# TINY-KE/DSP-SLAM-RGBD

Hardware: AMD Instinct MI355X
Metric: object-reconstructions/sec (2048 pts, 10 GN iters) (higher is better)
Workload: dtype fp16-mfma: 3xFP16 split (hi/lo fp16, fp32 accumulate) for every value that reaches an output + one-product fp16 classification of ray samples

## Files before the change

### dsp-slam-rgbd_amd/csrc/dsr_api.hip

```cpp
#include <hip/hip_runtime.h>
#include <rccl/rccl.h>
#include <dlfcn.h>

#include <algorithm>
#include <chrono>
#include <climits>
#include <cmath>
#include <cstdio>
#include <cstring>
#include <functional>
#include <map>
#include <mutex>
#include <string>
#include <thread>
#include <vector>

#include "../../include/dsr.h"
#include "dsr_kernels.hpp"
#include "dsr_mc.hpp"
#include "dsr_mesh.hpp"

#ifndef DSR_DEFAULT_FWD_VARIANT
#define DSR_DEFAULT_FWD_VARIANT 12
#endif
// ... 1443 lines not shown
  if (timing) DSR_CHECK(ctx, hipEventRecord(b->ev[0], ctx->stream));
  hipLaunchKernelGGL(k_init_state, dim3(n), dim3(64), 0, ctx->stream, n, b->t_in, b->is_oc, b->z_in, b->st,
                     b->zbuf, b->iters);
  DSR_CHECK(ctx, hipMemsetAsync(b->diag, 0, sizeof(int) * STD_INTS, ctx->stream));
  if (b->n_tied) DSR_CHECK(ctx, hipMemsetAsync(b->fail_view, 0xff, sizeof(int) * b->n_tied, ctx->stream));
  if (b->tie_multi)
    for (const auto& gr : b->groups)
      hipLaunchKernelGGL(k_views_pose, dim3(gr.nt), dim3(64), 0, ctx->stream, (const int2*)b->tie + gr.t0,
                         b->st + gr.o0, (const float*)b->cview + (size_t)gr.o0 * 16);
  b->spare_run = false;
  return batch_enqueue_iters(b, timing, 0, b->iters);
}

static int batch_redo(dsr_batch* b) {
  dsr_ctx* ctx = b->ctx;
  if (b->loop_iters <= b->iters || b->spare_run) return 0;
  std::vector<ObjState> hs(b->n_obj);
  DSR_CHECK(ctx, hipMemcpy(hs.data(), b->st, sizeof(ObjState) * hs.size(), hipMemcpyDeviceToHost));
  bool any = false;
  for (const ObjState& o : hs) any = any || (o.status == ST_RUNNING && o.lite_redo);
  if (!any) return 0;
  b->spare_run = true;
  const int rc = batch_enqueue_iters(b, b->timed, b->iters, b->loop_iters);
  if (rc) return rc;
  DSR_CHECK(ctx, hipEventRecord(b->done_ev, ctx->stream));
  return 1;
}
static int batch_finish(dsr_batch* b) {
  dsr_ctx* ctx = b->ctx;
  std::lock_guard<std::recursive_mutex> run(ctx->run_mu);
  DSR_CHECK(ctx, hipStreamSynchronize(ctx->stream));
  const int rc = batch_redo(b);
  if (rc < 0) return rc;
  if (rc == 1) DSR_CHECK(ctx, hipStreamSynchronize(ctx->stream));
  return 0;
}

static int batch_enqueue_iters(dsr_batch* b, bool timing, int it0, int it1) {
  dsr_ctx* ctx = b->ctx;
  hipStream_t s0 = ctx->stream;
  const int n = b->n_obj;
  const DevDecoder& D = b->dec->D;
  const GNParams P = b->P;
  const int grid = ctx->n_cu;
  const int cb = (n + 63) / 64;
  const int fv = fwd_variant();
  const FwdKernel fwdk = fwd_kernel_for(D, fv);
  const JacKernel jack = jac_kernel_for(D);
  const LiteKernel litek = lite_kernel();
  {
    const int fl = fv & 15;
    const bool known = fl == 1 || fl == 2 || fl == 3 || fl == 6 || fl == 7 || fl == 8 || fl == 12;
    const int jv = jac_variant();
    b->ran_fwd = is_variant(D) ? 12 : (known ? fv : (fv & ~15));
    b->ran_jac = is_variant(D) ? 12 : ((jv == 8 || jv == 12) ? jv : 0);
    b->ran_lite = b->lite ? lite_variant_dispatched() : 0;
    b->ran_ring = is_variant(D) ? 2 : split_ring();
  }
  const int np = (int)b->passes.size() - 1;
  const size_t epi = ev_per_iter(b);
  const int G = (int)b->groups.size();
  DSR_CHECK(ctx, hipEventRecord(b->fork_ev, s0));
  for (int g = 1; g < G; ++g) DSR_CHECK(ctx, hipStreamWaitEvent(ctx->gstream[g], b->fork_ev, 0));
  for (int it = it0; it < it1; ++it) {
    for (int g = 0; g < G; ++g) {
      const dsr_batch::Group& gr = b->groups[g];
      hipStream_t s = ctx->gstream[g];
      const int ng = gr.n, o0 = gr.o0;
      const ObjDesc* desc = b->desc + o0;
      ObjState* st = b->st + o0;
      float* zbuf = b->zbuf + (size_t)o0 * CODE;
      float* b0 = b->bias0f + (size_t)o0 * HID;
      float* b4 = b->bias4f + (size_t)o0 * HID;
      hipEvent_t* ev = b->ev.data() + 2 + ((size_t)it * G + g) * epi;
      hipLaunchKernelGGL(k_iter_begin, dim3(ng), dim3(512), 0, s, ng, desc, st, zbuf, D, P, b0, b4, b->dobs);
      ErtArgs ert = b->lite_cfg;
      ert.dead = b->dead;
      ert.M = b->M;
      ert.nth = -P.cut_off;
      ert.st = b->lite ? st : nullptr;
      ert.refine = b->refine;
      ert.diag = b->diag;
      const bool chunked = b->prescan && gr.n_rch > 0;
      if (!chunked)
        DSR_CHECK(ctx, hipMemsetD32Async(reinterpret_cast<hipDeviceptr_t>(b->dense + gr.c0), 0x7fc00000,
                                         (size_t)(gr.c1 - gr.c0), s));
      for (int pz = 0; pz < np; ++pz) {
        const int ra = b->passes[pz], rb = b->passes[pz + 1];
        if (chunked) {
          if (pz == 0)
            hipLaunchKernelGGL(k_sample_scan, dim3(gr.n_rch), dim3(RENDER_RAYS), 0, s, gr.rchunks, desc, st, b->rays,
                               b->M, rb, b->dead, b->rinfo, b->rwin, gr.scnt, b->dense);
          else
            hipLaunchKernelGGL(k_sample_count, dim3(gr.n_rch), dim3(RENDER_RAYS), 0, s, gr.rchunks, desc, st, b->rays,
                               b->M, ra, rb, b->dead, b->rinfo, b->rwin, gr.scnt);
          hipLaunchKernelGGL(k_sample_emit, dim3(gr.n_rch + 1), dim3(RENDER_RAYS), 0, s, gr.rchunks, desc, st,
                             b->rays, b->M, ra, rb, b->cand, b->rwin, gr.scnt,
                             ChunkTiles{gr.och, gr.tiles_f, gr.nt_f, ng, b->lite ? LTILE : TILE, 0});
        } else {
          hipLaunchKernelGGL(k_sample_pass, dim3(ng), dim3(SAMPLE_THREADS), 0, s, ng, desc, st, b->rays, b->M,
                             ra, rb, b->cand, b->dead, b->rinfo);
          hipLaunchKernelGGL(k_tiles_fwd, dim3(1), dim3(1024), 0, s, ng, desc, st, gr.tiles_f, gr.nt_f,
                             b->lite ? LTILE : TILE, 0);
        }
        if (fv & 1) DSR_CHECK(ctx, hipMemsetAsync(gr.sync, 0, 8 * 32 * sizeof(unsigned), s));
        if (timing) DSR_CHECK(ctx, hipEventRecord(ev[2 * pz], s));
        if (b->lite)
          hipLaunchKernelGGL(litek, dim3(grid), dim3(512), 0, s, D, gr.tiles_f, gr.nt_f, desc,
                             b->cand, b0, b4, b->dense, ert);
        else
          hipLaunchKernelGGL(fwdk, dim3(grid), dim3(512), 0, s, D, gr.tiles_f, gr.nt_f, desc, b->cand,
                             b0, b4, b->dense, gr.sync, ert, MaskArgs{nullptr, nullptr, nullptr, nullptr});
        if (timing) DSR_CHECK(ctx, hipEventRecord(ev[2 * pz + 1], s));
      }
      const bool rays = gr.n_rch > 0;
      if (b->lite) {
        if (rays) {
          hipLaunchKernelGGL(k_refine_scan, dim3(gr.n_rch), dim3(REFINE_SCAN_THREADS), 0, s, gr.rchunks, desc, st, b->M,
                             b->refine, refine_all() ? nullptr : b->dense, -P.cut_off, b->rbits, b->abits, gr.ccnt,
                             b->ma.slotmap);
          const int wp = (b->ma.pts && fv == 12) ? 1 : 0;
          hipLaunchKernelGGL(k_refine_emit, dim3(gr.n_rch + (chunked ? 1 : 0)), dim3(RENDER_RAYS), 0, s, gr.rchunks,
                             desc, st, b->rays, b->M, b->cand, b->ma.slotmap, b->rbits, b->abits, gr.ccnt,
                             chunked ? ChunkTiles{gr.och, gr.tiles_f, gr.nt_f, ng, TILE, wp} : ChunkTiles{});
        }
        if (!chunked)
          hipLaunchKernelGGL(k_tiles_fwd, dim3(1), dim3(1024), 0, s, ng, desc, st, gr.tiles_f, gr.nt_f, TILE,
                             (b->ma.pts && fv == 12) ? 1 : 0);
        if (timing) DSR_CHECK(ctx, hipEventRecord(ev[2 * np], s));
        const ErtArgs ex{nullptr, b->M, -P.cut_off, st, nullptr};
        if (b->ma.msk && fv == 12)
          hipLaunchKernelGGL(fwd16_kernel<512>(), dim3(grid), dim3(512), 0, s, D, gr.tiles_f, gr.nt_f, desc,
                             b->cand, b0, b4, b->dense, gr.sync, ex, b->ma);
        else
          hipLaunchKernelGGL(fwdk, dim3(grid), dim3(512), 0, s, D, gr.tiles_f, gr.nt_f, desc, b->cand,
                             b0, b4, b->dense, gr.sync, ex, MaskArgs{nullptr, nullptr, nullptr, nullptr});
        if (timing) DSR_CHECK(ctx, hipEventRecord(ev[2 * np + 1], s));
      }
      const bool keep = b->lite && b->ma.msk && fv == 12;
      const int je = 2 * (np + (b->lite ? 1 : 0));
      if (rays) {
        hipLaunchKernelGGL(k_render_rays, dim3(gr.n_rch), dim3(RENDER_RAYS), render_lds_bytes(b->M), s,
                           gr.rchunks, desc, st, b->rays, b->dobs, P, b->dense, b->kst, b->rst,
                           keep ? b->sst : nullptr, (const int*)b->ma.slotmap, gr.ccnt);
        hipLaunchKernelGGL(k_render_gather, dim3(gr.n_rch + (chunked ? 1 : 0)), dim3(256), 0, s, gr.rchunks, desc,
                           st, gr.ccnt, b->M, b->kst, b->rst, b->sst, b->kpts, b->kres, keep ? b->kslot : nullptr,
                           chunked ? ChunkTiles{gr.och, gr.tiles_j, gr.nt_j, ng, TILE, 0} : ChunkTiles{});
      }
      if (!chunked)
        hipLaunchKernelGGL(k_tiles_jac, dim3(1), dim3(1024), 0, s, ng, desc, st, gr.tiles_j, gr.nt_j);
      if (timing) DSR_CHECK(ctx, hipEventRecord(ev[je], s));
      hipLaunchKernelGGL(jack, dim3(grid), dim3(512), 0, s, D, gr.tiles_j, gr.nt_j, desc, st,
                         b->pts, b->kpts, b->kres, b0, b4, P, b->slots,
                         (const float4*)nullptr, (float*)nullptr, (float*)nullptr,
                         keep ? b->ma : MaskArgs{nullptr, nullptr, nullptr, nullptr},
                         D.ln_mask ? ctx->lnws[g] : (float*)nullptr);
      if (timing) DSR_CHECK(ctx, hipEventRecord(ev[je + 1], s));
      float* sred = b->sred + (size_t)o0 * SRED_STRIDE;
      hipLaunchKernelGGL(k_reduce_slots, dim3(ng * SLOT_BLOCKS), dim3(256), 0, s, desc, st, b->slots, sred, it,
                         b->counts + (size_t)o0 * COUNT_STRIDE, n);
      if (b->n_tied) {
        hipLaunchKernelGGL(k_solve_views, dim3(gr.nt), dim3(SOLVE_THREADS), 0, s, (const int2*)b->tie + gr.t0, desc,
                           st, zbuf, P, sred, b->tr_H ? b->tr_H + (size_t)o0 * TRACE_H_STRIDE : nullptr,
                           b->tr_v ? b->tr_v + (size_t)o0 * TRACE_V_STRIDE : nullptr,
                           b->tr_i ? b->tr_i + (size_t)o0 * TRACE_I_STRIDE : nullptr, n, b->fail_view + gr.t0);
        if (b->tie_multi)
          hipLaunchKernelGGL(k_views_pose, dim3(gr.nt), dim3(64), 0, s, (const int2*)b->tie + gr.t0, st,
                             (const float*)b->cview + (size_t)o0 * 16);
        continue;
      }
      hipLaunchKernelGGL(k_solve, dim3(ng), dim3(SOLVE_THREADS), 0, s, ng, desc, st, zbuf, P, sred,
                         b->tr_H ? b->tr_H + (size_t)o0 * TRACE_H_STRIDE : nullptr,
                         b->tr_v ? b->tr_v + (size_t)o0 * TRACE_V_STRIDE : nullptr,
                         b->tr_i ? b->tr_i + (size_t)o0 * TRACE_I_STRIDE : nullptr, n);
    }
  }
  for (int g = 1; g < G; ++g) {
    DSR_CHECK(ctx, hipEventRecord(b->join_ev[g], ctx->gstream[g]));
    DSR_CHECK(ctx, hipStreamWaitEvent(s0, b->join_ev[g], 0));
  }
  hipLaunchKernelGGL(k_finalize, dim3(cb), dim3(64), 0, s0, n, b->st, b->zbuf, b->out);
  DSR_CHECK(ctx, hipGetLastError());
  if (timing) DSR_CHECK(ctx, hipEventRecord(b->ev[1], s0));
  return 0;
// ... 1345 lines not shown
```

### dsp-slam-rgbd_amd/csrc/dsr_kernels.hpp

```cpp
#pragma once
#include "dsr_dev.hpp"
#include "dsr_mlp.hpp"
#include "dsr_mlp16.hpp"
#include "dsr_mlp_lite.hpp"
#include "../../include/dsr.h"

extern "C" __device__ __attribute__((const)) unsigned long long __ockl_wfred_max_u64(unsigned long long);

namespace dsr {

template <int N>
__device__ __forceinline__ void lu_small(float (&a)[N][N], int (&piv)[N]) {
#pragma unroll
  for (int k = 0; k < N; ++k) {
    int p = k;
    float best = fabsf(a[k][k]);
#pragma unroll
    for (int r = k + 1; r < N; ++r)
      if (fabsf(a[r][k]) > best) { best = fabsf(a[r][k]); p = r; }
    piv[k] = p;
#pragma unroll
    for (int r = k + 1; r < N; ++r) {
      const bool sw = (p == r);
#pragma unroll
// ... 537 lines not shown
        cnt = walk_count(make_float3(rp[0], rp[1], rp[2]), L, M, ra, rb, true, nin);
      }
    }
    rwin[d.ray_off + ray] = cnt | ((j0 + 1) << 8);
#ifdef DSR_EXP_PROV
    prov_alive(S.iters_done, ra, d.ray_off + ray, alive ? cnt + 1 : -1);
    prov_emit(S.iters_done, ra, d.ray_off + ray, cnt > 0 ? (j0 >= 0 ? j0 + ra : -2) : -1);
#endif
  }
  chunk_sums(cnt, 0, sc + 2 * blockIdx.x);
}

__global__ __launch_bounds__(RENDER_RAYS) DSR_NO_PK_F32 void k_sample_emit(const RenderChunk* __restrict__ chunks,
                                                             const ObjDesc* __restrict__ desc, ObjState* st,
                                                             const float* __restrict__ rays_all, int M, int ra,
                                                             int rb, float4* __restrict__ cand,
                                                             const int* __restrict__ rwin,
                                                             const int* __restrict__ sc, ChunkTiles T) {
  if (T.och && (int)blockIdx.x == (int)gridDim.x - 1) {
    chunk_tiles_fwd(T, desc, st, sc, 2, ra == 0 ? sc + 1 : nullptr);
    return;
  }
  const RenderChunk ch = chunks[blockIdx.x];
  ObjState& S = st[ch.obj];
  if (S.status != ST_RUNNING) return;
  const ObjDesc d = desc[ch.obj];
  __shared__ int wsum[RENDER_RAYS / 64];
  __shared__ SampleLds L;
  const int tid = threadIdx.x, lane = tid & 63, wv = tid >> 6;
  stage_samples(L, S, M, tid);
  const bool last = (int)blockIdx.x == ch.first + ch.n - 1;
  const int base = block_chunk_sum(sc, 2, ch.first, blockIdx.x);
  const int nin = (last && ra == 0) ? block_chunk_sum(sc + 1, 2, ch.first, blockIdx.x + 1) : 0;
  const int ray = ch.ray0 + tid;
  int cnt = 0, j0 = -1;
  float3 rv = make_float3(0.f, 0.f, 0.f);
  if (ray < d.n_rays) {
    const int w = rwin[d.ray_off + ray];
    cnt = w & 255;
    j0 = (w >> 8) - 1;
    if (cnt > 0) {
      const float* rp = rays_all + (size_t)(d.ray_off + ray) * 3;
      rv = make_float3(rp[0], rp[1], rp[2]);
    }
  }
  const int inc = wave_incl_scan(cnt, lane);
  if (lane == 63) wsum[wv] = inc;
  __syncthreads();
  int off = d.cand_off + base + inc - cnt;
  for (int k = 0; k < wv; ++k) off += wsum[k];
  if (cnt > 0 && j0 >= 0) {
    for (int k = ra; k < ra + cnt; ++k) {
      const float3 x = ray_sample(rv, L, j0 + k);
      cand[off++] = make_float4(x.x, x.y, x.z, __int_as_float(ray * M + j0 + k));
    }
  } else if (cnt > 0) {
    int rank = 0;
    for (int j = 0; j < M && rank < rb; ++j) {
      const float3 x = ray_sample(rv, L, j);
      const float nrm = sqrtf((x.x * x.x + x.y * x.y) + x.z * x.z);
      if (!(nrm < 1.0f)) continue;
      if (rank >= ra) cand[off++] = make_float4(x.x, x.y, x.z, __int_as_float(ray * M + j));
      ++rank;
    }
  }
  if (tid == 0 && last) {
    int t = base;
    for (int k = 0; k < RENDER_RAYS / 64; ++k) t += wsum[k];
    S.n_emit = t;
    S.n_eval += t;
    if (ra == 0) {
      S.n_valid = nin;
      if (nin < 10) {
        S.status = ST_FAIL;
        S.fail_reason = DSR_FAIL_RENDER_FEW;
      }
    }
  }
}

__global__ __launch_bounds__(SAMPLE_THREADS) DSR_NO_PK_F32 void k_sample_pass(int n_obj, const ObjDesc* __restrict__ desc,
                                                                ObjState* st, const float* __restrict__ rays_all,
                                                                int M, int ra, int rb, float4* __restrict__ cand,
                                                                int* __restrict__ dead, int* __restrict__ rinfo) {
  const int o = blockIdx.x;
  ObjState& S = st[o];
  if (S.status != ST_RUNNING) return;
  const ObjDesc d = desc[o];
  const float* rays = rays_all + (size_t)d.ray_off * 3;
  const bool first = ra == 0;
  __shared__ int wsum[SAMPLE_THREADS / 64];
  __shared__ int wnin[SAMPLE_THREADS / 64];
  __shared__ int base_s, nin_s;
  __shared__ SampleLds L;
  const int tid = threadIdx.x, lane = tid & 63, wv = tid >> 6;
  if (tid == 0) { base_s = 0; nin_s = 0; }
  stage_samples(L, S, M, tid);
  __syncthreads();
  for (int r0 = 0; r0 < d.n_rays; r0 += SAMPLE_THREADS) {
    const int ray = r0 + tid;
    int cnt = 0, nin = 0;
    int j0 = -1;
    float3 rv = make_float3(0.f, 0.f, 0.f);
    if (ray < d.n_rays) {
      rv = make_float3(rays[ray * 3 + 0], rays[ray * 3 + 1], rays[ray * 3 + 2]);
      if (first) dead_put(dead + d.ray_off + ray, 0);
      const bool alive = first || dead_get(dead + d.ray_off + ray) == 0;
      if (alive && !first) {
        const int info = rinfo[d.ray_off + ray];
        if (info >= 0) {
          j0 = info & 255;
          nin = info >> 8;
          cnt = max(0, min(rb, nin) - ra);
        }
      }
      if (alive && j0 < 0) {
        if (first) {
          int rank = 0, jf = -1, jl = -1;
          for (int j = 0; j < M; ++j) {
            const float3 x = ray_sample(rv, L, j);
            const float nrm = sqrtf((x.x * x.x + x.y * x.y) + x.z * x.z);
            if (!(nrm < 1.0f)) continue;
            if (jf < 0) jf = j;
            jl = j;
            if (rank < rb) ++cnt;
            ++rank;
          }
          nin = rank;
          rinfo[d.ray_off + ray] = rank == 0 ? 0 : (jl - jf + 1 == rank ? (jf | (rank << 8)) : -1);
        } else {
          cnt = walk_count(rv, L, M, ra, rb, true, nin);
        }
      }
    }
    const int inc = wave_incl_scan(cnt, lane);
    int nin_w = nin;
#pragma unroll
    for (int k = 32; k > 0; k >>= 1) nin_w += __shfl_xor(nin_w, k);
    if (lane == 63) wsum[wv] = inc;
    if (lane == 0) wnin[wv] = nin_w;
    __syncthreads();
    int off = base_s + inc - cnt;
    for (int k = 0; k < wv; ++k) off += wsum[k];
    if (cnt > 0 && j0 >= 0) {
      for (int k = ra; k < ra + cnt; ++k) {
        const float3 x = ray_sample(rv, L, j0 + k);
        cand[d.cand_off + off++] = make_float4(x.x, x.y, x.z, __int_as_float(ray * M + j0 + k));
      }
    } else if (cnt > 0) {
      int rank = 0;
      for (int j = 0; j < M && rank < rb; ++j) {
        const float3 x = ray_sample(rv, L, j);
        const float nrm = sqrtf((x.x * x.x + x.y * x.y) + x.z * x.z);
        if (!(nrm < 1.0f)) continue;
        if (rank >= ra) cand[d.cand_off + off++] = make_float4(x.x, x.y, x.z, __int_as_float(ray * M + j));
        ++rank;
      }
    }
    __syncthreads();
    if (tid == 0) {
      int t = 0, u = 0;
      for (int k = 0; k < SAMPLE_THREADS / 64; ++k) { t += wsum[k]; u += wnin[k]; }
      base_s += t;
      nin_s += u;
    }
    __syncthreads();
  }
  if (tid == 0) {
    S.n_emit = base_s;
    S.n_eval += base_s;
    if (first) {
// ... 657 lines not shown
  const int w = __builtin_amdgcn_readfirstlane(threadIdx.x >> 6);
  float* const lnw = lnws ? lnws + (size_t)blockIdx.x * LN_WS_WG : nullptr;
  const int nt = *n_tiles;
#ifdef DSR_EXP_STAMP
  unsigned long long jstamp[8] = {0, 0, 0, 0, 0, 0, 0, 0};
  unsigned long long jstamp_last = __builtin_amdgcn_s_memtime();
  int jtiles = 0;
#endif
  for (int ti = blockIdx.x; ti < nt; ti += gridDim.x) {
    const Tile tl = tiles[ti];
    const ObjDesc d = desc[tl.obj];
#ifdef DSR_EXP_STAMP
    ++jtiles;
#endif
    float zpre = 0.f;
    {
      const int tid = opaque(threadIdx.x);
      if (tid < TILE) {
        float x = 0.f, y = 0.f, z = 0.f, aux = 0.f, rr = 0.f;
        zpre = bias0f[tl.obj * HID];
        if (tid < tl.count) {
          if (tl.term == 0) {
            const float* p = pts_all + (size_t)(d.pts_off + tl.start + tid) * 3;
            const float3 xo = xform(st[tl.obj].T, p[0], p[1], p[2]);
            x = xo.x; y = xo.y; z = xo.z;
          } else if (tl.term == 1) {
            const float4 v = kpts[d.cand_off + tl.start + tid];
            x = v.x; y = v.y; z = v.z; aux = v.w;
            rr = kres[d.cand_off + tl.start + tid];
          } else {
            const float4 v = raw_pts[tl.start + tid];
            x = v.x; y = v.y; z = v.z;
          }
        }
        *reinterpret_cast<float4*>(sm.xyz + tid * 4) = make_float4(x, y, z, aux);
        sm.r[tid] = rr;
      }
    }
    __syncthreads();
    uint64_t mk[8];
    float v[4][4][4];
    floatx4 acc[4][4];
    int sa;
    Scales2 fs;
    bool fast = false;
    if (MA.kslot != nullptr && tl.term == 1) {
      const int tid = opaque(threadIdx.x);
      int bad = 0;
      if (tid < tl.count) bad = MA.kslot[d.cand_off + tl.start + tid] < 0;
      fast = !__syncthreads_or(bad);
    } else if (MA.pts != nullptr && tl.term == 0) {
      fast = true;
    }
    auto mslot = [&](int p) {
      return tl.term == 1 ? d.cand_off + MA.kslot[d.cand_off + tl.start + p] : MA.surf_base + d.pts_off + tl.start + p;
    };
    if (fast) {
      const int lane = opaque(threadIdx.x & 63), g = lane >> 4, c = lane & 15;
#pragma unroll
      for (int l = 0; l < 8; ++l) mk[l] = 0;
#pragma unroll
      for (int cb = 0; cb < 4; ++cb) {
        const int p = 16 * cb + c;
        if (p < tl.count) {
          const uint4 m4 = *reinterpret_cast<const uint4*>(MA.msk + (size_t)mslot(p) * 256 + (w * 4 + g) * 8);
          const unsigned dw[4] = {m4.x, m4.y, m4.z, m4.w};
#pragma unroll
          for (int l = 0; l < 8; ++l) {
            const unsigned u = (dw[l >> 1] >> (16 * (l & 1))) & 0xFFFFu;
#pragma unroll
            for (int q = 0; q < 4; ++q) mk[l] |= (uint64_t)((u >> (4 * q)) & 0xFu) << (16 * q + 4 * cb);
          }
        }
      }
      const int tid = opaque(threadIdx.x);
      if (tid < TILE) sm.y[tid] = (tid < tl.count) ? MA.yv[mslot(tid)] : 0.f;
      __syncthreads();
      JSTAMP(0)
    } else {
      JSTAMP(0)
      {
        const int lane = opaque(threadIdx.x & 63), g = lane >> 4, c = lane & 15;
        const float* bias0 = bias0f + tl.obj * HID;
        float m = 0.f;
        mk[0] = 0;
#pragma unroll
        for (int q = 0; q < 4; ++q) {
          const int n0 = 64 * w + 16 * q + 4 * g;
          const float4 bb = *reinterpret_cast<const float4*>(bias0 + n0);
          float wx[12];
#pragma unroll
          for (int i = 0; i < 12; ++i) wx[i] = D.W0x[n0 * 3 + i];
#pragma unroll
          for (int cb = 0; cb < 4; ++cb) {
            const float4 p = *reinterpret_cast<const float4*>(sm.xyz + (16 * cb + c) * 4);
#pragma unroll
            for (int r = 0; r < 4; ++r)
              v[q][cb][r] = fetch4(bb, r) + ((wx[3 * r] * p.x + wx[3 * r + 1] * p.y) + wx[3 * r + 2] * p.z);
          }
        }
        if (VAR && (D.ln_mask & 1)) ln_fwd(v, D.ln_g[0], D.ln_b[0], D.ln_dim[0], sm.red, sm.red2, w, lane, lnw);
#pragma unroll
        for (int q = 0; q < 4; ++q)
#pragma unroll
          for (int cb = 0; cb < 4; ++cb)
#pragma unroll
            for (int r = 0; r < 4; ++r) {
              const float h = fmaxf(v[q][cb][r], 0.f);
              if (h > 0.f) mk[0] |= 1ull << ((q * 4 + cb) * 4 + r);
              v[q][cb][r] = h;
              m = fmaxf(m, h);
            }
        if (VAR && D.xyz_all && w == 7) xyz_rows(v, sm.xyz, lane, m, 3);
        JSTAMP(7)
        fs = block_scale2(m, sm.wmax, w, lane);
        JSTAMP(3)
        write_split(v, fs.of(w), sm.Hh, sm.Hl, w, lane);
        JSTAMP(4)
      }
      __syncthreads();
      JSTAMP(5)
#pragma unroll 1
      for (int l = 1; l <= 6; ++l) {
        const int lane = opaque(threadIdx.x & 63), g = lane >> 4;
        gemm16_sel<PRIO, NB, JFWD_LS>(D.Wh_raw[l], w, D.Kf[l] / 32, sm.Hh, sm.Hl, acc, lane, fs.resc());
        JSTAMP(1)
        const float usc = ldexpf(1.f, -(D.sw[l] + fs.b));
        const float* bias = (l == 4) ? bias4f + tl.obj * HID : D.bias[l];
        float m = 0.f;
        uint64_t bits = 0;
        if (VAR && ((D.ln_mask >> l) & 1)) {
#pragma unroll
          for (int q = 0; q < 4; ++q) {
            const float4 bb = *reinterpret_cast<const float4*>(bias + 64 * w + 16 * q + 4 * g);
#pragma unroll
            for (int cb = 0; cb < 4; ++cb)
#pragma unroll
              for (int r = 0; r < 4; ++r) v[q][cb][r] = __builtin_fmaf(accr(acc[q][cb], r), usc * rc_sign(q, cb), fetch4(bb, r));
          }
          ln_fwd(v, D.ln_g[l], D.ln_b[l], D.ln_dim[l], sm.red, sm.red2, w, lane, lnw + (size_t)l * LN_WS_LAYER);
#pragma unroll
          for (int q = 0; q < 4; ++q)
#pragma unroll
            for (int cb = 0; cb < 4; ++cb)
#pragma unroll
              for (int r = 0; r < 4; ++r) {
                const float h = fmaxf(v[q][cb][r], 0.f);
                if (h > 0.f) bits |= 1ull << ((q * 4 + cb) * 4 + r);
                v[q][cb][r] = h;
                m = fmaxf(m, h);
              }
        } else {
#pragma unroll
        for (int q = 0; q < 4; ++q) {
          const float4 bb = *reinterpret_cast<const float4*>(bias + 64 * w + 16 * q + 4 * g);
#pragma unroll
          for (int cb = 0; cb < 4; ++cb) {
#pragma unroll
            for (int r = 0; r < 4; ++r) {
              const float h = fmaxf(__builtin_fmaf(accr(acc[q][cb], r), usc * rc_sign(q, cb), fetch4(bb, r)), 0.f);
              if (h > 0.f) bits |= 1ull << ((q * 4 + cb) * 4 + r);
              v[q][cb][r] = h;
              m = fmaxf(m, h);
            }
          }
        }
        }
        mk[l] = bits;
        {
          const int xr = VAR ? xyz_row(D, l) : (l == 3 ? D.l3 : -1);
          if (xr >= 0 && w == (xr >> 6)) xyz_rows(v, sm.xyz, lane, m, (xr >> 4) & 3);
        }
        JSTAMP(2)
        fs = block_scale2(m, sm.wmax, w, lane);
        JSTAMP(3)
        write_split(v, fs.of(w), sm.Hh, sm.Hl, w, lane);
        JSTAMP(4)
        __syncthreads();
        JSTAMP(5)
      }
      {
        const int lane = opaque(threadIdx.x & 63);
        gemm16_sel<PRIO, NB, JFWD_LS>(D.Wh_raw[7], w, D.Kf[7] / 32, sm.Hh, sm.Hl, acc, lane, fs.resc());
        JSTAMP(1)
        const int un = D.sw[7] + fs.b;
#pragma unroll
        for (int q = 0; q < 4; ++q)
#pragma unroll
          for (int cb = 0; cb < 4; ++cb)
#pragma unroll
            for (int r = 0; r < 4; ++r) acc[q][cb][r] = ldexpf(acc[q][cb][r], -un) * rc_sign(q, cb);
        const bool ln7 = VAR && ((D.ln_mask >> 7) & 1);
        if (ln7) ln_l7(acc, D, sm.red, sm.red2, w, lane, lnw + (size_t)7 * LN_WS_LAYER);
        epi_l7(acc, D, sm.red, w, lane, mk[7], VAR ? sm.xyz : nullptr, !ln7);
      }
      __syncthreads();
      {
        const int tid = opaque(threadIdx.x);
        if (tid < TILE) {
          float s = sm.red[tid];
          for (int k = 1; k < NWAVE; ++k) s += sm.red[k * TILE + tid];
          float y = tanhf(s + D.b8);
          if (VAR && D.use_tanh) y = tanhf(y);
          sm.y[tid] = y;
        }
      }
      __syncthreads();
    }
    float xg[4][3] = {{0.f, 0.f, 0.f}, {0.f, 0.f, 0.f}, {0.f, 0.f, 0.f}, {0.f, 0.f, 0.f}};
    const bool xlane = VAR && D.xyz_all && w == 7 && ((threadIdx.x & 63) >> 4) == 3;
    {
      const int lane = opaque(threadIdx.x & 63), g = lane >> 4, c = lane & 15;
      float m = 0.f;
#pragma unroll
      for (int q = 0; q < 4; ++q) {
        const int n0 = 64 * w + 16 * q + 4 * g;
        const float4 w8 = *reinterpret_cast<const float4*>(D.W8 + n0);
#pragma unroll
        for (int cb = 0; cb < 4; ++cb) {
          const int p = 16 * cb + c;
          const float yy = sm.y[p];
          float dt = 1.f - yy * yy;
          if (VAR && D.use_tanh) {
            const float t = atanhf(yy);
            dt = dt * (1.f - t * t);
          }
#pragma unroll
          for (int r = 0; r < 4; ++r) {
            const float gv = ((mk[7] >> ((q * 4 + cb) * 4 + r)) & 1ull) ? dt * fetch4(w8, r) : 0.f;
            v[q][cb][r] = gv;
            m = fmaxf(m, fabsf(gv));
            if (q == 3 && r >= 1 && xlane) xg[cb][r - 1] = dt * fetch4(w8, r);
          }
        }
      }
      if (VAR && ((D.ln_mask >> 7) & 1))
        m = ln_bwd(v, D.ln_g[7], D.ln_dim[7], sm.red, sm.red2, w, lane, lnw + (size_t)7 * LN_WS_LAYER);
      JSTAMP(7)
      sa = block_scale(m, sm.wmax, w, lane);
      JSTAMP(3)
      write_split(v, sa, sm.Hh, sm.Hl, w, lane);
      JSTAMP(4)
    }
    __syncthreads();
    JSTAMP(5)
#pragma unroll 1
    for (int l = 7; l >= 1; --l) {
      const int lane = opaque(threadIdx.x & 63), g = lane >> 4, c = lane & 15;
      gemm16_sel<PRIO, NB, BWD_LS>(D.Wbh_raw[l], w, D.Kb[l] / 32, sm.Hh, sm.Hl, acc, lane);
      JSTAMP(1)
      const float usc = ldexpf(1.f, -(D.swb[l] + sa));
// ... 755 lines not shown
```

### dsp-slam-rgbd_amd/csrc/dsr_mlp16.hpp

```cpp
#pragma once
#include <utility>
#include "dsr_dev.hpp"
#include "dsr_mlp.hpp"

namespace dsr {

typedef _Float16 half8 __attribute__((ext_vector_type(8)));
typedef _Float16 half4 __attribute__((ext_vector_type(4)));

constexpr int PH = 528;

#if defined(DSR_LITE_EXPERIMENTS) || defined(DSR_EXP_NOSIGN)
constexpr bool SPLIT_ROW_SIGNS = false;
#else
constexpr bool SPLIT_ROW_SIGNS = true;
#endif
__device__ __forceinline__ constexpr float row_sign(int q) { return (SPLIT_ROW_SIGNS && (q & 1)) ? -1.f : 1.f; }
#ifdef DSR_EXP_COLSIGN
__device__ __forceinline__ constexpr float col_sign(int cb) { return (SPLIT_ROW_SIGNS && (cb & 1)) ? -1.f : 1.f; }
#else
__device__ __forceinline__ constexpr float col_sign(int) { return 1.f; }
#endif
__device__ __forceinline__ constexpr float rc_sign(int q, int cb) { return row_sign(q) * col_sign(cb); }

// ... 330 lines not shown
};
__device__ __forceinline__ Scales2 block_scale2(float m, float* wmax, int w, int lane) {
  m = wave_max(m, lane);
  if (lane == 0) wmax[w] = m;
  __syncthreads();
  float ma = wmax[0], mb = wmax[4];
#pragma unroll
  for (int k = 1; k < 4; ++k) {
    ma = fmaxf(ma, wmax[k]);
    mb = fmaxf(mb, wmax[4 + k]);
  }
  return Scales2{group_scale_exp(ma), group_scale_exp(mb)};
}

typedef float float2v __attribute__((ext_vector_type(2)));
typedef _Float16 half2v __attribute__((ext_vector_type(2)));

__device__ __forceinline__ void write_split(const float (&v)[4][4][4], int s, _Float16* Hh, _Float16* Hl,
                                            int w, int lane) {
  const int c = lane & 15, g = (lane >> 4) ^ (((c >> 2) & 1) << 1);
#pragma unroll
  for (int q = 0; q < 4; ++q) {
    const int n0 = 64 * w + 16 * q + 4 * g;
#pragma unroll
    for (int cb = 0; cb < 4; ++cb) {
      const int p = 16 * cb + c;
      half4 hh, hl;
      const float2v sc2 = float2v{1.f, 1.f} * (ldexpf(1.f, s) * col_sign(cb));
#pragma unroll
      for (int r = 0; r < 4; r += 2) {
        const float2v x = float2v{v[q][cb][r], v[q][cb][r + 1]} * sc2;
        const half2v h = __builtin_convertvector(x, half2v);
        hh[r] = h[0]; hh[r + 1] = h[1];
        const unsigned hb = __builtin_bit_cast(unsigned, h);
        unsigned lb;
        asm("v_fma_mixlo_f16 %0, -%1, 1.0, %2 op_sel_hi:[1,0,0]" : "=v"(lb) : "v"(hb), "v"(x[0]));
        asm("v_fma_mixhi_f16 %0, -%1, 1.0, %2 op_sel:[1,0,0] op_sel_hi:[1,0,0]" : "+v"(lb) : "v"(hb), "v"(x[1]));
        const half2v l = __builtin_bit_cast(half2v, lb);
        hl[r] = l[0]; hl[r + 1] = l[1];
      }
      *reinterpret_cast<half4*>(Hh + p * PH + n0) = hh;
      *reinterpret_cast<half4*>(Hl + p * PH + n0) = hl;
    }
  }
}

struct MaskQueue {
  unsigned d[4][4];
};

__device__ __forceinline__ void mask_push(MaskQueue& mq, uint64_t mk) {
#pragma unroll
  for (int cb = 0; cb < 4; ++cb) {
    unsigned u = 0;
#pragma unroll
    for (int q = 0; q < 4; ++q) u |= (unsigned)((mk >> (16 * q + 4 * cb)) & 0xFull) << (4 * q);
    mq.d[cb][0] = (mq.d[cb][0] >> 16) | (mq.d[cb][1] << 16);
    mq.d[cb][1] = (mq.d[cb][1] >> 16) | (mq.d[cb][2] << 16);
    mq.d[cb][2] = (mq.d[cb][2] >> 16) | (mq.d[cb][3] << 16);
    mq.d[cb][3] = (mq.d[cb][3] >> 16) | (u << 16);
  }
}

__device__ __forceinline__ void mask_store(const MaskQueue& mq, uint16_t* msk, int cand_base, int count, int w,
                                           int lane) {
  const int g = lane >> 4, c = lane & 15;
#pragma unroll
  for (int cb = 0; cb < 4; ++cb) {
    const int p = 16 * cb + c;
    if (p < count)
      *reinterpret_cast<uint4*>(msk + (size_t)(cand_base + p) * 256 + (w * 4 + g) * 8) =
          make_uint4(mq.d[cb][0], mq.d[cb][1], mq.d[cb][2], mq.d[cb][3]);
  }
}

template <int I>
__device__ __forceinline__ float keep_if(float a, uint64_t mask) {
  const unsigned word = (unsigned)(mask >> (I & 32));
  int m;
  asm("v_bfe_i32 %0, %1, %2, 1" : "=v"(m) : "v"(word), "i"(I & 31));
  return __int_as_float(__float_as_int(a) & m);
}

__device__ __forceinline__ uint64_t relu_bits(const float (&v)[4][4][4]) {
  uint64_t mk = 0;
#pragma unroll
  for (int q = 0; q < 4; ++q)
#pragma unroll
    for (int cb = 0; cb < 4; ++cb)
#pragma unroll
      for (int r = 0; r < 4; ++r)
        if (v[q][cb][r] > 0.f) mk |= 1ull << ((q * 4 + cb) * 4 + r);
  return mk;
}

template <int NCB>
__device__ __forceinline__ void xyz_rows(float (&v)[4][NCB][4], const float* xyz, int lane, float& m, int xq) {
  const int g = lane >> 4, c = lane & 15;
#pragma unroll
  for (int q = 0; q < 4; ++q) {
    if (q != xq) continue;
    const bool on = g == 3;
#pragma unroll
    for (int cb = 0; cb < NCB; ++cb) {
      const float4 p = *reinterpret_cast<const float4*>(xyz + (16 * cb + c) * 4);
      v[q][cb][1] = on ? p.x : v[q][cb][1];
      v[q][cb][2] = on ? p.y : v[q][cb][2];
      v[q][cb][3] = on ? p.z : v[q][cb][3];
      m = fmaxf(m, on ? fmaxf(fabsf(p.x), fmaxf(fabsf(p.y), fabsf(p.z))) : 0.f);
    }
  }
}

__device__ __forceinline__ void ln_point_sums(float (&s)[4], float* red, int w, int lane) {
  const int g = lane >> 4, c = lane & 15;
#pragma unroll
  for (int cb = 0; cb < 4; ++cb) {
    s[cb] += xor_lane(s[cb], lane, 16);
    s[cb] += xor_lane(s[cb], lane, 32);
    if (g == 0) red[w * 64 + 16 * cb + c] = s[cb];
  }
}
__device__ __forceinline__ float ln_total(const float* red, int cb, int c) {
  float t = red[16 * cb + c];
#pragma unroll
  for (int k = 1; k < NWAVE; ++k) t += red[k * 64 + 16 * cb + c];
  return t;
}

__device__ __forceinline__ void ln_fwd(float (&v)[4][4][4], const float* __restrict__ gam,
                                       const float* __restrict__ bet, int D, float* red, float* red2, int w,
                                       int lane, float* __restrict__ xh) {
  const int g = lane >> 4, c = lane & 15;
  float s[4] = {0.f, 0.f, 0.f, 0.f};
#pragma unroll
  for (int q = 0; q < 4; ++q)
#pragma unroll
    for (int cb = 0; cb < 4; ++cb)
#pragma unroll
      for (int r = 0; r < 4; ++r) s[cb] += (64 * w + 16 * q + 4 * g + r < D) ? v[q][cb][r] : 0.f;
  ln_point_sums(s, red, w, lane);
  __syncthreads();
  const float invD = 1.f / (float)D;
  float mean[4];
#pragma unroll
  for (int cb = 0; cb < 4; ++cb) {
    mean[cb] = ln_total(red, cb, c) * invD;
    s[cb] = 0.f;
  }
#pragma unroll
  for (int q = 0; q < 4; ++q)
#pragma unroll
    for (int cb = 0; cb < 4; ++cb)
#pragma unroll
      for (int r = 0; r < 4; ++r) {
        const float d = v[q][cb][r] - mean[cb];
        s[cb] += (64 * w + 16 * q + 4 * g + r < D) ? d * d : 0.f;
      }
  ln_point_sums(s, red2, w, lane);
  __syncthreads();
  float rstd[4];
#pragma unroll
  for (int cb = 0; cb < 4; ++cb) rstd[cb] = 1.f / sqrtf(ln_total(red2, cb, c) * invD + 1e-5f);
  const int tid = w * 64 + lane;
#pragma unroll
  for (int q = 0; q < 4; ++q) {
    const int n0 = 64 * w + 16 * q + 4 * g;
    const float4 gg = *reinterpret_cast<const float4*>(gam + n0);
    const float4 bb = *reinterpret_cast<const float4*>(bet + n0);
#pragma unroll
    for (int cb = 0; cb < 4; ++cb) {
      float xa[4];
#pragma unroll
      for (int r = 0; r < 4; ++r) {
        const bool live = n0 + r < D;
        xa[r] = live ? (v[q][cb][r] - mean[cb]) * rstd[cb] : 0.f;
// ... 7 lines not shown
#pragma unroll
    for (int cb = 0; cb < 4; ++cb) xh[16 * 512 * 4 + 16 * cb + c] = rstd[cb];
  }
}

__device__ __forceinline__ float ln_bwd(float (&v)[4][4][4], const float* __restrict__ gam, int D, float* red,
                                        float* red2, int w, int lane, const float* __restrict__ xh) {
  const int g = lane >> 4, c = lane & 15;
  const int tid = w * 64 + lane;
  float s1[4] = {0.f, 0.f, 0.f, 0.f}, s2[4] = {0.f, 0.f, 0.f, 0.f};
#pragma unroll
  for (int q = 0; q < 4; ++q) {
    const int n0 = 64 * w + 16 * q + 4 * g;
    const float4 gg = *reinterpret_cast<const float4*>(gam + n0);
#pragma unroll
    for (int cb = 0; cb < 4; ++cb) {
      const float4 x4 = *reinterpret_cast<const float4*>(xh + (size_t)((q * 4 + cb) * 512 + tid) * 4);
#pragma unroll
      for (int r = 0; r < 4; ++r) {
        const float gx = (n0 + r < D) ? v[q][cb][r] * fetch4(gg, r) : 0.f;
        s1[cb] += gx;
        s2[cb] += gx * fetch4(x4, r);
      }
    }
  }
  ln_point_sums(s1, red, w, lane);
  ln_point_sums(s2, red2, w, lane);
  __syncthreads();
  const float invD = 1.f / (float)D;
  float m1[4], m2[4], rs[4];
#pragma unroll
  for (int cb = 0; cb < 4; ++cb) {
    m1[cb] = ln_total(red, cb, c) * invD;
    m2[cb] = ln_total(red2, cb, c) * invD;
    rs[cb] = xh[16 * 512 * 4 + 16 * cb + c];
  }
  float m = 0.f;
#pragma unroll
  for (int q = 0; q < 4; ++q) {
    const int n0 = 64 * w + 16 * q + 4 * g;
    const float4 gg = *reinterpret_cast<const float4*>(gam + n0);
#pragma unroll
    for (int cb = 0; cb < 4; ++cb) {
      const float4 x4 = *reinterpret_cast<const float4*>(xh + (size_t)((q * 4 + cb) * 512 + tid) * 4);
#pragma unroll
      for (int r = 0; r < 4; ++r) {
        const bool live = n0 + r < D;
        const float gx = v[q][cb][r] * fetch4(gg, r);
        const float ga = live ? rs[cb] * ((gx - m1[cb]) - fetch4(x4, r) * m2[cb]) : 0.f;
        v[q][cb][r] = ga;
        m = fmaxf(m, fabsf(ga));
      }
    }
  }
  return m;
}

__device__ __forceinline__ void ln_l7(floatx4 (&acc)[4][4], const DevDecoder& D, float* red, float* red2, int w,
                                      int lane, float* __restrict__ xh) {
  float (&v)[4][4][4] = reinterpret_cast<float (&)[4][4][4]>(acc);
  const int g = lane >> 4;
#pragma unroll
  for (int q = 0; q < 4; ++q) {
    const float4 bb = *reinterpret_cast<const float4*>(D.bias[7] + 64 * w + 16 * q + 4 * g);
#pragma unroll
    for (int cb = 0; cb < 4; ++cb)
#pragma unroll
      for (int r = 0; r < 4; ++r) v[q][cb][r] = v[q][cb][r] + fetch4(bb, r);
  }
  ln_fwd(v, D.ln_g[7], D.ln_b[7], D.ln_dim[7], red, red2, w, lane, xh);
}

struct NoStamp {
  __device__ __forceinline__ void operator()(int) const {}
};

template <class Stamp = NoStamp>
__device__ __forceinline__ Scales2 epi16(floatx4 (&acc)[4][4], int unscale, const float* __restrict__ bias,
                                         Fwd16Shared& sm, int w, int lane, uint64_t& mk, int xr,
                                         Stamp stamp = Stamp{}, const DevDecoder* lnd = nullptr, int l = 0) {
  const int g = lane >> 4, c = lane & 15;
  const float usc = ldexpf(1.f, -unscale);
  float v[4][4][4];
  float m = 0.f;
  uint64_t bits = 0;
  if (lnd != nullptr && ((lnd->ln_mask >> l) & 1)) {
#pragma unroll
    for (int q = 0; q < 4; ++q) {
      const float4 bb = *reinterpret_cast<const float4*>(bias + 64 * w + 16 * q + 4 * g);
#pragma unroll
      for (int cb = 0; cb < 4; ++cb)
#pragma unroll
        for (int r = 0; r < 4; ++r) v[q][cb][r] = __builtin_fmaf(accr(acc[q][cb], r), usc * rc_sign(q, cb), fetch4(bb, r));
    }
    ln_fwd(v, lnd->ln_g[l], lnd->ln_b[l], lnd->ln_dim[l], sm.red, sm.red2, w, lane, nullptr);
#pragma unroll
    for (int q = 0; q < 4; ++q)
#pragma unroll
      for (int cb = 0; cb < 4; ++cb)
#pragma unroll
        for (int r = 0; r < 4; ++r) {
          const float x = fmaxf(v[q][cb][r], 0.f);
          if (x > 0.f) bits |= 1ull << ((q * 4 + cb) * 4 + r);
          v[q][cb][r] = x;
          m = fmaxf(m, x);
        }
  } else {
#pragma unroll
  for (int q = 0; q < 4; ++q) {
    const int n0 = 64 * w + 16 * q + 4 * g;
    const float4 bb = *reinterpret_cast<const float4*>(bias + n0);
#pragma unroll
    for (int cb = 0; cb < 4; ++cb) {
#pragma unroll
      for (int r = 0; r < 4; ++r) {
        const float x = fmaxf(__builtin_fmaf(accr(acc[q][cb], r), usc * rc_sign(q, cb), fetch4(bb, r)), 0.f);
        if (x > 0.f) bits |= 1ull << ((q * 4 + cb) * 4 + r);
        v[q][cb][r] = x;
        m = fmaxf(m, x);
      }
    }
  }
  }
  if (xr >= 0 && w == (xr >> 6)) xyz_rows(v, sm.xyz, lane, m, (xr >> 4) & 3);
  stamp(2);
  const Scales2 sc = block_scale2(m, sm.wmax, w, lane);
  stamp(3);
  write_split(v, sc.of(w), sm.Hh, sm.Hl, w, lane);
  stamp(4);
  mk = bits;
  return sc;
}

template <bool PRIO, int X>
__global__ __launch_bounds__(512) void k_mlp_fwd16(DevDecoder D, const Tile* __restrict__ tiles,
                                                   const int* __restrict__ n_tiles,
                                                   const ObjDesc* __restrict__ desc,
                                                   const float4* __restrict__ cand,
                                                   const float* __restrict__ bias0f,
                                                   const float* __restrict__ bias4f,
                                                   float* __restrict__ dense, unsigned* __restrict__,
                                                   ErtArgs E, MaskArgs MA) {
  __shared__ Fwd16Shared sm;
  const int w = __builtin_amdgcn_readfirstlane(threadIdx.x >> 6);
  const int nt = *n_tiles;
  constexpr bool MSK = (X & 512) != 0;
  constexpr bool VAR = (X & 8192) != 0;
  constexpr int NB = ((X >> 10) & 3) == 0 ? 0 : 1 + ((X >> 10) & 3);
#ifdef DSR_EXP_STAMP
  unsigned long long fst[12] = {0, 0, 0, 0, 0, 0, 0, 0, 0, 0, 0, 0};
  unsigned long long fst_last = __builtin_amdgcn_s_memtime();
  int ftiles = 0;
  auto stamp = [&](int cat) {
    __builtin_amdgcn_sched_barrier(0);
    const unsigned long long t = __builtin_amdgcn_s_memtime();
    fst[cat] += t - fst_last;
    fst_last = t;
    __builtin_amdgcn_sched_barrier(0);
  };
#else
  NoStamp stamp;
#endif
  for (int ti = blockIdx.x; ti < nt; ti += gridDim.x) {
#ifdef DSR_EXP_STAMP
    ++ftiles;
#endif
    const Tile tl = tiles[ti];
    const ObjDesc d = desc[tl.obj];
    const bool surf = MSK && tl.term == 3;
    const int mbase = surf ? MA.surf_base + d.pts_off + tl.start : d.cand_off + tl.start;
    float zpre = 0.f, ylpre = 0.f;
    {
      const int tid = opaque(threadIdx.x);
      if (tid < TILE) {
        float4 v = make_float4(0.f, 0.f, 0.f, 0.f);
        zpre = bias0f[tl.obj * HID];
        if (tid < tl.count) {
          if (surf) {
            const float* p = MA.pts + (size_t)(d.pts_off + tl.start + tid) * 3;
            const float3 xo = xform(E.st[tl.obj].T, p[0], p[1], p[2]);
            v = make_float4(xo.x, xo.y, xo.z, 0.f);
          } else {
            v = cand[d.cand_off + tl.start + tid];
            if (E.st) ylpre = dense[d.cand_off + (__float_as_int(v.w) & ~AUDIT_BIT)];
          }
        }
        *reinterpret_cast<float4*>(sm.xyz + tid * 4) = v;
      }
    }
    __syncthreads();
    stamp(0);
    Scales2 sa;
    MaskQueue mq;
    {
      const int lane = opaque(threadIdx.x & 63), g = lane >> 4, c = lane & 15;
      const float* bias0 = bias0f + tl.obj * HID;
      float v[4][4][4];
      float m = 0.f;
#pragma unroll
      for (int q = 0; q < 4; ++q) {
        const int n0 = 64 * w + 16 * q + 4 * g;
        const float4 bb = *reinterpret_cast<const float4*>(bias0 + n0);
        float wx[12];
#pragma unroll
        for (int i = 0; i < 12; ++i) wx[i] = D.W0x[n0 * 3 + i];
#pragma unroll
        for (int cb = 0; cb < 4; ++cb) {
          const float4 p = *reinterpret_cast<const float4*>(sm.xyz + (16 * cb + c) * 4);
#pragma unroll
          for (int r = 0; r < 4; ++r)
            v[q][cb][r] = fetch4(bb, r) + ((wx[3 * r] * p.x + wx[3 * r + 1] * p.y) + wx[3 * r + 2] * p.z);
        }
      }
      if (VAR && (D.ln_mask & 1)) ln_fwd(v, D.ln_g[0], D.ln_b[0], D.ln_dim[0], sm.red, sm.red2, w, lane, nullptr);
#pragma unroll
      for (int q = 0; q < 4; ++q)
#pragma unroll
        for (int cb = 0; cb < 4; ++cb)
#pragma unroll
          for (int r = 0; r < 4; ++r) {
            v[q][cb][r] = fmaxf(v[q][cb][r], 0.f);
            m = fmaxf(m, v[q][cb][r]);
          }
      uint64_t b0 = 0;
      if constexpr (MSK) b0 = relu_bits(v);
      if (VAR && D.xyz_all && w == 7) xyz_rows(v, sm.xyz, lane, m, 3);
      sa = block_scale2(m, sm.wmax, w, lane);
      write_split(v, sa.of(w), sm.Hh, sm.Hl, w, lane);
      if constexpr (MSK) mask_push(mq, b0);
    }
    __syncthreads();
    floatx4 acc[4][4];
#pragma unroll 1
    for (int l = 1; l <= 6; ++l) {
      const int lane = opaque(threadIdx.x & 63);
      stamp(7);
      if (SURF_LS != FWD_LS && surf) gemm16_sel<PRIO, NB, SURF_LS>(D.Wh_raw[l], w, D.Kf[l] / 32, sm.Hh, sm.Hl, acc, lane, sa.resc());
      else gemm16_sel<PRIO, NB, FWD_LS>(D.Wh_raw[l], w, D.Kf[l] / 32, sm.Hh, sm.Hl, acc, lane, sa.resc());
      stamp(1);
      uint64_t mk;
      sa = epi16(acc, D.sw[l] + sa.b, (l == 4) ? bias4f + tl.obj * HID : D.bias[l], sm, w, lane, mk,
                 VAR ? xyz_row(D, l) : (l == 3 ? D.l3 : -1), stamp, VAR ? &D : nullptr, l);
      if constexpr (MSK) mask_push(mq, mk);
      stamp(7);
      __syncthreads();
      stamp(5);
    }
    {
      const int lane = opaque(threadIdx.x & 63);
      stamp(7);
      if (SURF_LS != FWD_LS && surf) gemm16_sel<PRIO, NB, SURF_LS>(D.Wh_raw[7], w, D.Kf[7] / 32, sm.Hh, sm.Hl, acc, lane, sa.resc());
      else gemm16_sel<PRIO, NB, FWD_LS>(D.Wh_raw[7], w, D.Kf[7] / 32, sm.Hh, sm.Hl, acc, lane, sa.resc());
      stamp(1);
      const int un = D.sw[7] + sa.b;
#pragma unroll
      for (int q = 0; q < 4; ++q)
#pragma unroll
        for (int cb = 0; cb < 4; ++cb)
#pragma unroll
          for (int r = 0; r < 4; ++r) acc[q][cb][r] = ldexpf(acc[q][cb][r], -un) * rc_sign(q, cb);
      uint64_t mask;
      const bool ln7 = VAR && ((D.ln_mask >> 7) & 1);
      if (ln7) ln_l7(acc, D, sm.red, sm.red2, w, lane, nullptr);
      epi_l7(acc, D, sm.red, w, lane, mask, VAR ? sm.xyz : nullptr, !ln7);
      if constexpr (MSK) {
        mask_push(mq, mask);
        mask_store(mq, MA.msk, mbase, tl.count, w, lane);
      }
      stamp(8);
    }
    __syncthreads();
    stamp(9);
    {
      const int tid = opaque(threadIdx.x);
      float emax = 0.f;
      if (tid < tl.count) {
        float s = sm.red[tid];
        for (int k = 1; k < NWAVE; ++k) s += sm.red[k * TILE + tid];
        float y = tanhf(s + D.b8);
        if (VAR && D.use_tanh) y = tanhf(y);
        stamp(10);
        const float4 p = *reinterpret_cast<const float4*>(sm.xyz + tid * 4);
        const float zprobe = zpre;
        if (p.x != p.x || p.y != p.y || p.z != p.z || zprobe != zprobe) y = __builtin_nanf("");
        if (surf) {
          MA.yv[mbase + tid] = y;
        } else {
          const int tagged = __float_as_int(p.w);
          const int idx = tagged & ~AUDIT_BIT;
          if (E.st) {
            const float yl = ylpre;
            const float e = fabsf(y - yl);
            if (e == e) emax = e;
            if (tagged & AUDIT_BIT) {
              const int cl = yl <= E.nth ? 0 : (yl < -E.nth ? 1 : 2);
              const int ce = y <= E.nth ? 0 : (y < -E.nth ? 1 : 2);
              if (cl != ce) atomicAdd(&E.st[tl.obj].lite_viol, 1);
            }
          }
          dense[d.cand_off + idx] = y;
          if constexpr (MSK) MA.yv[d.cand_off + tl.start + tid] = y;
          if (E.dead && y <= E.nth) dead_put(E.dead + d.ray_off + idx / E.M, 1);
        }
      }
      stamp(11);
      if (w == 0 && E.st && !surf) {
        emax = wave_max(emax, opaque(threadIdx.x & 63));
        if ((threadIdx.x & 63) == 0 && emax > 0.f)
// ... 15 lines not shown
```

Baseline: 374.6.

## Fuse dense NaN fill into sample pass and use integer relu-mask/max asm

Measured after the change: 376.2 (median of 6 runs). No clear change (+0.4%).

```diff
diff --git a/dsp-slam-rgbd_amd/csrc/dsr_api.hip b/dsp-slam-rgbd_amd/csrc/dsr_api.hip
--- a/dsp-slam-rgbd_amd/csrc/dsr_api.hip
+++ b/dsp-slam-rgbd_amd/csrc/dsr_api.hip
@@ -1549,9 +1549,11 @@
       ert.refine = b->refine;
       ert.diag = b->diag;
       const bool chunked = b->prescan && gr.n_rch > 0;
+#ifdef DSR_EXP_FILLMEMSET
       if (!chunked)
         DSR_CHECK(ctx, hipMemsetD32Async(reinterpret_cast<hipDeviceptr_t>(b->dense + gr.c0), 0x7fc00000,
                                          (size_t)(gr.c1 - gr.c0), s));
+#endif
       for (int pz = 0; pz < np; ++pz) {
         const int ra = b->passes[pz], rb = b->passes[pz + 1];
         if (chunked) {
@@ -1566,7 +1568,7 @@
                              ChunkTiles{gr.och, gr.tiles_f, gr.nt_f, ng, b->lite ? LTILE : TILE, 0});
         } else {
           hipLaunchKernelGGL(k_sample_pass, dim3(ng), dim3(SAMPLE_THREADS), 0, s, ng, desc, st, b->rays, b->M,
-                             ra, rb, b->cand, b->dead, b->rinfo);
+                             ra, rb, b->cand, b->dead, b->rinfo, pz == 0 ? b->dense : (float*)nullptr);
           hipLaunchKernelGGL(k_tiles_fwd, dim3(1), dim3(1024), 0, s, ng, desc, st, gr.tiles_f, gr.nt_f,
                              b->lite ? LTILE : TILE, 0);
         }
diff --git a/dsp-slam-rgbd_amd/csrc/dsr_kernels.hpp b/dsp-slam-rgbd_amd/csrc/dsr_kernels.hpp
--- a/dsp-slam-rgbd_amd/csrc/dsr_kernels.hpp
+++ b/dsp-slam-rgbd_amd/csrc/dsr_kernels.hpp
@@ -643,11 +643,17 @@
 __global__ __launch_bounds__(SAMPLE_THREADS) DSR_NO_PK_F32 void k_sample_pass(int n_obj, const ObjDesc* __restrict__ desc,
                                                                 ObjState* st, const float* __restrict__ rays_all,
                                                                 int M, int ra, int rb, float4* __restrict__ cand,
-                                                                int* __restrict__ dead, int* __restrict__ rinfo) {
+                                                                int* __restrict__ dead, int* __restrict__ rinfo,
+                                                                float* __restrict__ dense) {
   const int o = blockIdx.x;
   ObjState& S = st[o];
+  const ObjDesc d = desc[o];
+  if (dense != nullptr) {
+    float* row = dense + d.cand_off;
+    const int ne = d.n_rays * M;
+    for (int e = threadIdx.x; e < ne; e += SAMPLE_THREADS) row[e] = __builtin_nanf("");
+  }
   if (S.status != ST_RUNNING) return;
-  const ObjDesc d = desc[o];
   const float* rays = rays_all + (size_t)d.ray_off * 3;
   const bool first = ra == 0;
   __shared__ int wsum[SAMPLE_THREADS / 64];
@@ -1471,8 +1477,6 @@
       {
         const int lane = opaque(threadIdx.x & 63), g = lane >> 4, c = lane & 15;
         const float* bias0 = bias0f + tl.obj * HID;
-        float m = 0.f;
-        mk[0] = 0;
 #pragma unroll
         for (int q = 0; q < 4; ++q) {
           const int n0 = 64 * w + 16 * q + 4 * g;
@@ -1489,17 +1493,17 @@
           }
         }
         if (VAR && (D.ln_mask & 1)) ln_fwd(v, D.ln_g[0], D.ln_b[0], D.ln_dim[0], sm.red, sm.red2, w, lane, lnw);
+        ReluMask rm;
 #pragma unroll
         for (int q = 0; q < 4; ++q)
 #pragma unroll
-          for (int cb = 0; cb < 4; ++cb)
-#pragma unroll
-            for (int r = 0; r < 4; ++r) {
-              const float h = fmaxf(v[q][cb][r], 0.f);
-              if (h > 0.f) mk[0] |= 1ull << ((q * 4 + cb) * 4 + r);
-              v[q][cb][r] = h;
-              m = fmaxf(m, h);
-            }
+          for (int cb = 0; cb < 4; ++cb) {
+#pragma unroll
+            for (int r = 0; r < 4; ++r) v[q][cb][r] = fmaxf(v[q][cb][r], 0.f);
+            rm.push4(v[q][cb], (q * 4 + cb) * 4);
+          }
+        mk[0] = rm.bits();
+        float m = rm.top();
         if (VAR && D.xyz_all && w == 7) xyz_rows(v, sm.xyz, lane, m, 3);
         JSTAMP(7)
         fs = block_scale2(m, sm.wmax, w, lane);
@@ -1516,8 +1520,7 @@
         JSTAMP(1)
         const float usc = ldexpf(1.f, -(D.sw[l] + fs.b));
         const float* bias = (l == 4) ? bias4f + tl.obj * HID : D.bias[l];
-        float m = 0.f;
-        uint64_t bits = 0;
+        ReluMask rm;
         if (VAR && ((D.ln_mask >> l) & 1)) {
 #pragma unroll
           for (int q = 0; q < 4; ++q) {
@@ -1531,14 +1534,11 @@
 #pragma unroll
           for (int q = 0; q < 4; ++q)
 #pragma unroll
-            for (int cb = 0; cb < 4; ++cb)
-#pragma unroll
-              for (int r = 0; r < 4; ++r) {
-                const float h = fmaxf(v[q][cb][r], 0.f);
-                if (h > 0.f) bits |= 1ull << ((q * 4 + cb) * 4 + r);
-                v[q][cb][r] = h;
-                m = fmaxf(m, h);
-              }
+            for (int cb = 0; cb < 4; ++cb) {
+#pragma unroll
+              for (int r = 0; r < 4; ++r) v[q][cb][r] = fmaxf(v[q][cb][r], 0.f);
+              rm.push4(v[q][cb], (q * 4 + cb) * 4);
+            }
         } else {
 #pragma unroll
         for (int q = 0; q < 4; ++q) {
@@ -1546,16 +1546,14 @@
 #pragma unroll
           for (int cb = 0; cb < 4; ++cb) {
 #pragma unroll
-            for (int r = 0; r < 4; ++r) {
-              const float h = fmaxf(__builtin_fmaf(accr(acc[q][cb], r), usc * rc_sign(q, cb), fetch4(bb, r)), 0.f);
-              if (h > 0.f) bits |= 1ull << ((q * 4 + cb) * 4 + r);
-              v[q][cb][r] = h;
-              m = fmaxf(m, h);
-            }
+            for (int r = 0; r < 4; ++r)
+              v[q][cb][r] = fmaxf(__builtin_fmaf(accr(acc[q][cb], r), usc * rc_sign(q, cb), fetch4(bb, r)), 0.f);
+            rm.push4(v[q][cb], (q * 4 + cb) * 4);
           }
         }
         }
-        mk[l] = bits;
+        mk[l] = rm.bits();
+        float m = rm.top();
         {
           const int xr = VAR ? xyz_row(D, l) : (l == 3 ? D.l3 : -1);
           if (xr >= 0 && w == (xr >> 6)) xyz_rows(v, sm.xyz, lane, m, (xr >> 4) & 3);
diff --git a/dsp-slam-rgbd_amd/csrc/dsr_mlp16.hpp b/dsp-slam-rgbd_amd/csrc/dsr_mlp16.hpp
--- a/dsp-slam-rgbd_amd/csrc/dsr_mlp16.hpp
+++ b/dsp-slam-rgbd_amd/csrc/dsr_mlp16.hpp
@@ -436,16 +436,30 @@
   return __int_as_float(__float_as_int(a) & m);
 }
 
+struct ReluMask {
+  unsigned w[2] = {0u, 0u};
+  int mi = 0;
+  __device__ __forceinline__ void push4(const float (&x)[4], int K0) {
+#pragma unroll
+    for (int r = 0; r < 4; ++r) {
+      unsigned one;
+      asm("v_min_u32 %0, 1, %1" : "=v"(one) : "v"(__float_as_uint(x[r])));
+      asm("v_lshl_or_b32 %0, %1, %2, %0" : "+v"(w[(K0 + r) >> 5]) : "v"(one), "i"((K0 + r) & 31));
+    }
+    asm("v_max3_i32 %0, %0, %1, %2" : "+v"(mi) : "v"(__float_as_int(x[0])), "v"(__float_as_int(x[1])));
+    asm("v_max3_i32 %0, %0, %1, %2" : "+v"(mi) : "v"(__float_as_int(x[2])), "v"(__float_as_int(x[3])));
+  }
+  __device__ __forceinline__ uint64_t bits() const { return ((uint64_t)w[1] << 32) | w[0]; }
+  __device__ __forceinline__ float top() const { return __int_as_float(mi); }
+};
+
 __device__ __forceinline__ uint64_t relu_bits(const float (&v)[4][4][4]) {
-  uint64_t mk = 0;
+  ReluMask rm;
 #pragma unroll
   for (int q = 0; q < 4; ++q)
 #pragma unroll
-    for (int cb = 0; cb < 4; ++cb)
-#pragma unroll
-      for (int r = 0; r < 4; ++r)
-        if (v[q][cb][r] > 0.f) mk |= 1ull << ((q * 4 + cb) * 4 + r);
-  return mk;
+    for (int cb = 0; cb < 4; ++cb) rm.push4(v[q][cb], (q * 4 + cb) * 4);
+  return rm.bits();
 }
 
 template <int NCB>
@@ -619,8 +633,7 @@
   const int g = lane >> 4, c = lane & 15;
   const float usc = ldexpf(1.f, -unscale);
   float v[4][4][4];
-  float m = 0.f;
-  uint64_t bits = 0;
+  ReluMask rm;
   if (lnd != nullptr && ((lnd->ln_mask >> l) & 1)) {
 #pragma unroll
     for (int q = 0; q < 4; ++q) {
@@ -634,14 +647,11 @@
 #pragma unroll
     for (int q = 0; q < 4; ++q)
 #pragma unroll
-      for (int cb = 0; cb < 4; ++cb)
-#pragma unroll
-        for (int r = 0; r < 4; ++r) {
-          const float x = fmaxf(v[q][cb][r], 0.f);
-          if (x > 0.f) bits |= 1ull << ((q * 4 + cb) * 4 + r);
-          v[q][cb][r] = x;
-          m = fmaxf(m, x);
-        }
+      for (int cb = 0; cb < 4; ++cb) {
+#pragma unroll
+        for (int r = 0; r < 4; ++r) v[q][cb][r] = fmaxf(v[q][cb][r], 0.f);
+        rm.push4(v[q][cb], (q * 4 + cb) * 4);
+      }
   } else {
 #pragma unroll
   for (int q = 0; q < 4; ++q) {
@@ -651,21 +661,20 @@
     for (int cb = 0; cb < 4; ++cb) {
 #pragma unroll
       for (int r = 0; r < 4; ++r) {
-        const float x = fmaxf(__builtin_fmaf(accr(acc[q][cb], r), usc * rc_sign(q, cb), fetch4(bb, r)), 0.f);
-        if (x > 0.f) bits |= 1ull << ((q * 4 + cb) * 4 + r);
-        v[q][cb][r] = x;
-        m = fmaxf(m, x);
-      }
-    }
-  }
-  }
+        v[q][cb][r] = fmaxf(__builtin_fmaf(accr(acc[q][cb], r), usc * rc_sign(q, cb), fetch4(bb, r)), 0.f);
+      }
+      rm.push4(v[q][cb], (q * 4 + cb) * 4);
+    }
+  }
+  }
+  float m = rm.top();
   if (xr >= 0 && w == (xr >> 6)) xyz_rows(v, sm.xyz, lane, m, (xr >> 4) & 3);
   stamp(2);
   const Scales2 sc = block_scale2(m, sm.wmax, w, lane);
   stamp(3);
   write_split(v, sc.of(w), sm.Hh, sm.Hl, w, lane);
   stamp(4);
-  mk = bits;
+  mk = rm.bits();
   return sc;
 }
 
@@ -733,7 +742,6 @@
       const int lane = opaque(threadIdx.x & 63), g = lane >> 4, c = lane & 15;
       const float* bias0 = bias0f + tl.obj * HID;
       float v[4][4][4];
-      float m = 0.f;
 #pragma unroll
       for (int q = 0; q < 4; ++q) {
         const int n0 = 64 * w + 16 * q + 4 * g;
@@ -750,17 +758,17 @@
         }
       }
       if (VAR && (D.ln_mask & 1)) ln_fwd(v, D.ln_g[0], D.ln_b[0], D.ln_dim[0], sm.red, sm.red2, w, lane, nullptr);
+      ReluMask rm;
 #pragma unroll
       for (int q = 0; q < 4; ++q)
 #pragma unroll
-        for (int cb = 0; cb < 4; ++cb)
-#pragma unroll
-          for (int r = 0; r < 4; ++r) {
-            v[q][cb][r] = fmaxf(v[q][cb][r], 0.f);
-            m = fmaxf(m, v[q][cb][r]);
-          }
-      uint64_t b0 = 0;
-      if constexpr (MSK) b0 = relu_bits(v);
+        for (int cb = 0; cb < 4; ++cb) {
+#pragma unroll
+          for (int r = 0; r < 4; ++r) v[q][cb][r] = fmaxf(v[q][cb][r], 0.f);
+          rm.push4(v[q][cb], (q * 4 + cb) * 4);
+        }
+      float m = rm.top();
+      const uint64_t b0 = rm.bits();
       if (VAR && D.xyz_all && w == 7) xyz_rows(v, sm.xyz, lane, m, 3);
       sa = block_scale2(m, sm.wmax, w, lane);
       write_split(v, sa.of(w), sm.Hh, sm.Hl, w, lane);
```
